# bobocode/lmono

Hardware: AMD Instinct MI355X
Metric: KITTI HDL-64 scans/sec (scanRegistration + laserOdometry) (higher is better)
Workload: dtype f32 features / f64 solve

## Files before the change

### lmono_amd/csrc/corr_flat.hip

```cpp
#include "batch.hpp"

namespace lmono {

#ifndef LMONO_CF_T
#define LMONO_CF_T 128
#endif
constexpr int kCfT = LMONO_CF_T;
constexpr int kCfBlocks = kMaxQueries / kCfT;
static_assert(kMaxQueries % kCfT == 0, "feature capacity must be a multiple of the workgroup size");
static_assert(kCfBlocks == kThinBlocks, "k_lm_solve skips the records of the workgroups a thinned lead-in pair does not run");
#ifndef LMONO_CF_PER
#define LMONO_CF_PER 6
#endif
#ifndef LMONO_CF_WAVES
#define LMONO_CF_WAVES 1
#endif
constexpr int kCfPer = LMONO_CF_PER;
constexpr int kCfPool = kCfT * kCfPer;
#ifndef LMONO_R0_PLANE
#define LMONO_R0_PLANE 0.25f
#define LMONO_R0_EDGE 0.7f
#endif
constexpr float kCfR0Edge = LMONO_R0_EDGE, kCfR0Plane = LMONO_R0_PLANE;
constexpr int kCfC = 4;
// ... 9 lines not shown
constexpr int kCfNnRounds = LMONO_CF_NN_ROUNDS, kCfWalkRounds = LMONO_CF_WALK_ROUNDS;
#ifndef LMONO_CF_MERGED
#define LMONO_CF_MERGED 0
#endif
#ifndef LMONO_WALK_TIGHT
#define LMONO_WALK_TIGHT 1
#endif

__device__ __forceinline__ unsigned int cf_request_line(int line, int b0, int nb, int owner) { return (unsigned int)line | ((unsigned int)b0 << 7) | ((unsigned int)nb << 16) | ((unsigned int)owner << 25); }
static_assert(kCfT <= 128 && kAzBins <= 511, "request packing");

struct CfRun {
    unsigned int start;
    unsigned int pre;
    unsigned short len;
    unsigned char owner;
    unsigned char tag;
};
static_assert(sizeof(CfRun) == 12, "run descriptor layout");

struct CfLds {
    float4 elev[2][66];
    int fge[2][66], lle[2][66];
    float4 q[kCfT];
    unsigned long long best[kCfT];
    unsigned long long same[kCfT], other[kCfT];
    int closest[kCfT], wlo[kCfT], whi[kCfT];
    unsigned int req[kCfPool];
    CfRun pool[kCfPool];
    int n_pool, n_cand, wsum[kCfT / 64];
    unsigned char wmode[kCfT];
};

__device__ __forceinline__ void cf_defer(unsigned int *wl, int c, int qi)
{
    const unsigned int slot = atomicAdd(wl, 1u);
    wl[1 + slot] = ((unsigned int)c << 12) | (unsigned int)qi;
}

struct CfArc { int a0, nb; };
__device__ __forceinline__ void cf_arc(float r, float rho, float th, CfArc &a)
{
    constexpr float kb = kAzBins / 6.28318531f;
    a.a0 = 0; a.nb = kAzBins;
    if (!(rho > r * 1.002f)) return;
    const float alpha = asin_upper(r / rho) + kArcSlackBins / kb;
    const int lo = (int)floorf((th - alpha) * kb), hi = (int)floorf((th + alpha) * kb);
    const int n = hi - lo + 1;
    if (n >= kAzBins) return;
    a.a0 = ((lo % kAzBins) + kAzBins) % kAzBins;
    a.nb = n;
}
__device__ __forceinline__ int cf_arc_pieces(const CfArc &a) { return a.a0 + a.nb > kAzBins ? 2 : 1; }
__device__ __forceinline__ void cf_post_line(unsigned int *req, int &slot, const CfArc &a, int line, int owner)
{
    const int n0 = min(a.nb, kAzBins - a.a0);
    req[slot++] = cf_request_line(line, a.a0, n0, owner);
    if (n0 < a.nb) req[slot++] = cf_request_line(line, 0, a.nb - n0, owner);
}

__device__ __forceinline__ int cf_first_line(const float4 *el, float ehi)
{
    int lo = 0, hi = 66;
    while (lo < hi) { const int mid = (lo + hi) >> 1; if (el[mid].z <= ehi) hi = mid; else lo = mid + 1; }
    return lo;
}
__device__ __forceinline__ int cf_last_line(const float4 *el, float elo)
{
    int lo = -1, hi = 65;
    while (lo < hi) { const int mid = (lo + hi + 1) >> 1; if (el[mid].w >= elo) lo = mid; else hi = mid - 1; }
// ... 136 lines not shown
                    const unsigned long long key = ((unsigned long long)__float_as_uint(d) << 32) | seq;
                    const bool is_other = sj > 0 ? (dv > 0) : (dv < 0);
                    m1 = (ok & is_other & (key < m1)) ? key : m1;
                    m0 = (ok & !is_other & (key < m0)) ? key : m0;
                }
            }
        }
        CF_STAMP(cf_acc[13])
        if (!more) break;
    }
    flush();
    CF_STAMP(cf_acc[14])
}

__global__ __launch_bounds__(kCfT, LMONO_CF_WAVES) void k_corr_flat(BatchView b, OdomView o, int step, int outer, unsigned int *wl, int defer_every, unsigned long long *stats)
{
    __shared__ CfLds L;
    const int xcd = blockIdx.x & 7, u = blockIdx.x >> 3;
    const int ci = o.chain0 + (u / kCfBlocks) * 8 + xcd;
    const int qb = u % kCfBlocks;
    if (ci >= o.chain1) return;
    const int c = o.clist ? o.clist[ci] : ci;
    int own;
    const int k = chain_scan(o, c, step, own);
    if (k < 0) return;
    if (lead_in_thinned(o, k, own) && qb % kThinStride != 0) return;
    const int tid = threadIdx.x;
    const int l = k - 1;
    const int n_sharp = b.feat_n[k * 4 + 0];
    const int nq = n_sharp + b.feat_n[k * 4 + 2];
    if (qb >= nq) return;
    const int qi = tid * kCfBlocks + qb;
    if (b.status[l] & (kStatusIrregularLines | kStatusDenseCell)) {
        if (qi < nq) cf_defer(wl, c, qi);
        return;
    }
    const bool edge = qi < n_sharp;
    const int cl = edge ? 0 : 1;
    const int n_edge_owner = n_sharp > qb ? (n_sharp - qb + kCfBlocks - 1) / kCfBlocks : 0;
    float4 fp = make_float4(0.f, 0.f, 0.f, 0.f);
    int *seed_c = o.seed ? o.seed + (size_t)c * kMaxQueries : nullptr;
    int sidx = -1;
    if (qi < nq) {
        fp = edge ? b.sharp[(size_t)k * kMaxSharp + qi] : b.flat[(size_t)k * kMaxFlat + (qi - n_sharp)];
        if (outer == 1 && seed_c) sidx = seed_c[qi];
    }
    int4 prev = make_int4(-1, -1, -1, 0);
    if (qi < nq && outer == 1 && seed_c && sidx >= 0) prev = ((const int4 *)o.corr + (size_t)c * kMaxQueries)[qi];
    for (int xx = tid; xx < 2 * 66; xx += kCfT) {
        const int tc = xx / 66, v = xx % 66;
        L.elev[tc][v] = b.lb_elev[(size_t)(l * 2 + tc) * 66 + v];
        L.fge[tc][v] = b.line_first_ge[(size_t)(l * 2 + tc) * 66 + v];
        L.lle[tc][v] = b.line_last_le[(size_t)(l * 2 + tc) * 66 + v];
    }
    const int n_last = b.feat_n[l * 4 + (edge ? 1 : 3)];
    const float4 *cloud = edge ? b.less_sharp + (size_t)l * kMaxLessSharp : b.less_flat + b.off[l];
    float4 sp = make_float4(0.f, 0.f, 0.f, 0.f);
    if (sidx >= 0 && sidx < n_last) sp = cloud[sidx]; else sidx = -1;
    const double *x = o.state + c * 8;
    double rx, ry, rz;
    quat_rotate(x, (double)fp.x, (double)fp.y, (double)fp.z, rx, ry, rz);
    const float qx = (float)(rx + x[4]), qy = (float)(ry + x[5]), qz = (float)(rz + x[6]);
    float sd = -1.0f;
    if (sidx >= 0) { const float d = dist2f(sp.x, sp.y, sp.z, qx, qy, qz); if (d < 24.0f) sd = d; }
    L.q[tid] = make_float4(qx, qy, qz, 0.f);
    L.best[tid] = ~0ull;
    const int *tg_c = b.lb_start + (size_t)(l * 2 + 0) * (kLineKeys + 1), *tg_s = b.lb_start + (size_t)(l * 2 + 1) * (kLineKeys + 1);
// ... 249 lines not shown
                const unsigned long long lim = pack_fu(r_now * r_now * 0.998f, 0u);
                if (other < lim && (edge || same < lim)) walking = false;
                else if (seeded) r_seed = -1.0f;
                else {
                    wpass++;
                    while (wpass < 4 && rad[wpass] <= rad[wpass - 1]) wpass++;
#if LMONO_WALK_TIGHT
                    if (other < thr && (edge || same < thr)) {
                        const float d = edge ? __uint_as_float((unsigned int)(other >> 32)) : fmaxf(__uint_as_float((unsigned int)(other >> 32)), __uint_as_float((unsigned int)(same >> 32)));
                        const float rt = sqrtf(d) * 1.002f + 1e-3f;
                        if (wpass < 4 && rt < rad[wpass] && d < 24.0f) r_seed = rt;
                    }
#endif
                }
            }
        }
        CF_STAMP(cf_acc[3])
        if (!__syncthreads_or(walking ? 1 : 0)) break;
    }
#endif
#ifdef LMONO_TILE_PROF
    {
        const int mr = __syncthreads_or(0) * 0 + my_rounds;
        __shared__ int s_maxr, s_sumr;
        if (tid == 0) { s_maxr = 0; s_sumr = 0; }
        __syncthreads();
        atomicMax(&s_maxr, mr); atomicAdd(&s_sumr, mr);
        __syncthreads();
        if (tid == 0) { cf_acc[17] = (unsigned long long)s_maxr; cf_acc[18] = (unsigned long long)s_sumr; }
    }
    if (tid == 0 && stats) { atomicAdd(&stats[1], 1ull); for (int i = 0; i < 20; i++) atomicAdd(&stats[2 + i], cf_acc[i]); }
#endif
    if (qi >= nq) return;
    if (deferred || walking) { cf_defer(wl, c, qi); return; }
    int4 rres = make_int4(-1, -1, -1, 0);
    int closest_out = -1;
    if (n_last > 0 && nn != ~0ull && (double)__uint_as_float((unsigned int)(nn >> 32)) < 25.0) {
        closest_out = closest;
        const int i_other = other < thr ? seq_to_index((unsigned int)(other & 0xffffffffull), closest) : -1;
        if (edge) { if (i_other >= 0) rres = make_int4(closest, i_other, -1, 1); }
        else {
            const int i_same = same < thr ? seq_to_index((unsigned int)(same & 0xffffffffull), closest) : -1;
            if (i_same >= 0 && i_other >= 0) rres = make_int4(closest, i_same, i_other, 2);
        }
    }
    ((int4 *)o.corr + (size_t)c * kMaxQueries)[qi] = rres;
    if (outer == 0 && seed_c) seed_c[qi] = closest_out;
    float4 A = make_float4(0.f, 0.f, 0.f, 0.f), B = A, C = A;
    if (rres.w != 0) { A = cloud[rres.x]; B = cloud[rres.y]; if (rres.z >= 0) C = cloud[rres.z]; }
    fp.w = __int_as_float(rres.w);
    float4 *rec = o.crec + ((size_t)c * kMaxQueries + qi) * 4;
    rec[0] = fp; rec[1] = A; rec[2] = B; rec[3] = C;
}

}
```

### lmono_amd/csrc/lidar_abi.hip

```cpp
#pragma once
constexpr int kListGrid = 256;

struct lmono_scan_batch {
    lmono_ctx *ctx = nullptr;
    int n_cap = 0;
    int64_t pts_cap = 0;
    int n_scans = 0;
    int64_t total = 0;
    int max_pts = 0;
    bool registered = false;
    bool grid_built = false;
    std::vector<int64_t> off_h;
    bool validation_pending = false;
    std::vector<void *> allocs;
    BatchView v{};
    int64_t *off_d = nullptr;
    float *in_owned = nullptr;
    hipEvent_t staged_ev = nullptr, in_free_ev = nullptr;
    int64_t staged_points = -1;
    std::vector<int> feat_h;
    int chains_cap = 0;
    double *state = nullptr, *incr = nullptr, *poses = nullptr, *xq = nullptr;
    int *corr = nullptr, *lm_info = nullptr, *corr_pair = nullptr, *seed = nullptr;
    float4 *crec = nullptr, *crec_pair = nullptr;
// ... 282 lines not shown
    switch (which) {
    case 0: HIP_TRY(c, hipMemcpy(&n, b->v.n_cloud + scan, sizeof(int), hipMemcpyDeviceToHost)); src = b->v.cloud + b->off_h[scan]; break;
    case 1: n = fn[0]; src = b->v.sharp + (size_t)scan * kMaxSharp; break;
    case 2: n = fn[1]; src = b->v.less_sharp + (size_t)scan * kMaxLessSharp; break;
    case 3: n = fn[2]; src = b->v.flat + (size_t)scan * kMaxFlat; break;
    default: n = fn[3]; src = b->v.less_flat + b->off_h[scan]; break;
    }
    if (n > cap) { c->err = "get_cloud: output capacity too small"; return LMONO_ECAPACITY; }
    if (n > 0) HIP_TRY(c, hipMemcpy(out_h, src, sizeof(float4) * n, hipMemcpyDeviceToHost));
    return n;
}

extern "C" int lmono_batch_get_curvature(lmono_ctx *c, lmono_scan_batch *b, int scan, float *curv_h, int32_t *label_h, int cap)
{
    if (!c || !b || !b->registered || scan < 0 || scan >= b->n_scans) return LMONO_EINVAL;
    HIP_TRY(c, hipStreamSynchronize(c->stream));
    int n = 0;
    HIP_TRY(c, hipMemcpy(&n, b->v.n_cloud + scan, sizeof(int), hipMemcpyDeviceToHost));
    if (n > cap) { c->err = "get_curvature: output capacity too small"; return LMONO_ECAPACITY; }
    if (curv_h && n > 0) HIP_TRY(c, hipMemcpy(curv_h, b->v.curv + b->off_h[scan], sizeof(float) * n, hipMemcpyDeviceToHost));
    if (label_h && n > 0) {
        std::vector<int8_t> tmp(n);
        HIP_TRY(c, hipMemcpy(tmp.data(), b->v.label + b->off_h[scan], n, hipMemcpyDeviceToHost));
        for (int i = 0; i < n; i++) label_h[i] = tmp[i];
    }
    return n;
}

static int ensure_odom_ws(lmono_ctx *c, lmono_scan_batch *b, int n_chains)
{
    if (n_chains <= b->chains_cap) return LMONO_OK;
    bool ok = dalloc(b, b->state, (size_t)n_chains * 8) && dalloc(b, b->corr, (size_t)n_chains * kMaxQueries * 4) &&
              dalloc(b, b->lm_info, (size_t)n_chains * 4) && dalloc(b, b->crec, (size_t)n_chains * kMaxQueries * 4) &&
              dalloc(b, b->seed, (size_t)n_chains * kMaxQueries) && dalloc(b, b->wl, 8 * ((size_t)n_chains * kMaxQueries + 1)) &&
              dalloc(b, b->ws, (size_t)n_chains * 8) && dalloc(b, b->resid_d, (size_t)n_chains) && dalloc(b, b->rstat, (size_t)n_chains * 4) &&
              dalloc(b, b->rcount, (size_t)n_chains + 2);
    if (!ok) { c->err = "odometry workspace: hipMalloc failed"; return LMONO_ENOMEM; }
    b->chains_cap = n_chains;
    return LMONO_OK;
}

static int ensure_grid(lmono_ctx *c, lmono_scan_batch *b)
{
    if (b->grid_built) return LMONO_OK;
#ifdef LMONO_DIAG_SEARCH
    hipLaunchKernelGGL(k_grid_build, dim3(b->n_scans, 1 + kGridPar), dim3(1024), kGridLds, c->stream, b->v);
    int rc = check_launch(c, "k_grid_build");
    if (rc) return rc;
    b->grid_built = true; b->v.has_grid = 1;
    return LMONO_OK;
#else
    c->err = "the hash-grid searches exist in the diagnostic build only (-DLMONO_DIAG_SEARCH)";
    return LMONO_EINVAL;
#endif
}

struct GroupFork {
    lmono_ctx *c; int G, g_own; bool forked = false;
    GroupFork(lmono_ctx *c_, int G_, int g_own_) : c(c_), G(G_), g_own(g_own_) {}
    int fork()
    {
        if (G <= 1) return LMONO_OK;
        for (int g = g_own; g < G; g++)
            if (!c->gstream[g]) {
                int lo = 0, hi = 0;
                if (c->odom_prio && hipDeviceGetStreamPriorityRange(&lo, &hi) == hipSuccess) HIP_TRY(c, hipStreamCreateWithPriority(&c->gstream[g], hipStreamNonBlocking, hi));
                else HIP_TRY(c, hipStreamCreateWithFlags(&c->gstream[g], hipStreamNonBlocking));
// ... 6 lines not shown
    }
    int join()
    {
        if (!forked) return LMONO_OK;
        forked = false;
        int rc = LMONO_OK;
        for (int g = g_own; g < G; g++) {
            if (hipEventRecord(c->gev[g + 1], c->gstream[g]) != hipSuccess || hipStreamWaitEvent(c->stream, c->gev[g + 1], 0) != hipSuccess) {
                (void)hipStreamSynchronize(c->gstream[g]);
                c->err = "odometry: joining a chain-group stream failed"; rc = LMONO_ENODEV;
            }
        }
        return rc;
    }
    ~GroupFork() { (void)join(); }
};

static int odom_groups(const lmono_ctx *c, int n_ch)
{
    constexpr int kMinChainsPerGroup = 32;
    int G = c->opt[LMONO_OPT_ODOM_STREAMS];
    G = G < 1 ? 1 : (G > 8 ? 8 : G);
    if (c->stream != nullptr && G > 3 && !c->many_queues) G = 3;
    while (G > 1 && n_ch / G < kMinChainsPerGroup) G--;
    if (c->opt[LMONO_OPT_CORR_TILE] != 3) G = 1;
    return G;
}

static int odom_launch_steps(lmono_ctx *c, lmono_scan_batch *b, const OdomView &o, int n_ch, int step_a, int step_b, int G, EvSet *es, int *ne)
{
    const int tile = c->opt[LMONO_OPT_CORR_TILE];
    hipStream_t st = c->stream;
    const int g_own = st == nullptr ? 1 : 0;
    const size_t wl_stride = (size_t)b->chains_cap * kMaxQueries + 1;
    auto kev = [&](int i) -> hipEvent_t {
        if (!es) return nullptr;
        while ((int)es->kev.size() <= i) { hipEvent_t e; if (hipEventCreate(&e) != hipSuccess) return nullptr; es->kev.push_back(e); }
        return es->kev[i];
    };
    GroupFork fork(c, G, g_own);
    int rc = fork.fork();
    if (rc) return rc;
    for (int step = step_a; step < step_b; step++) {
        for (int outer = 0; outer < 2; outer++) {
            for (int g = 0; g < G; g++) {
                hipStream_t sg = (G == 1 || g < g_own) ? st : c->gstream[g];
                OdomView og = o;
                og.chain0 = (int)((long long)g * n_ch / G); og.chain1 = (int)((long long)(g + 1) * n_ch / G);
                const int ng = og.chain1 - og.chain0;
                if (ng <= 0) continue;
                unsigned int *wlg = b->wl + g * wl_stride;
                hipEvent_t e0 = nullptr, e1 = nullptr, e2 = nullptr;
                if (g == 0 && es) { e0 = kev(*ne); e1 = kev(*ne + 1); e2 = kev(*ne + 2); }
                if (e0 && e1 && e2) (void)hipEventRecord(e0, sg);
                if (tile == 3) {
                    hipLaunchKernelGGL(k_corr_flat, dim3(8 * ((ng + 7) / 8) * kCfBlocks), dim3(kCfT), 0, sg, b->v, og, step, outer, wlg, c->opt[LMONO_OPT_DEFER_EVERY], c->stats_d);
                    hipLaunchKernelGGL(k_correspond_list, dim3(kListGrid), dim3(256), 0, sg, b->v, og, step, outer, (const unsigned int *)wlg, c->stats_d);
                }
#ifdef LMONO_DIAG_SEARCH
                else
                    hipLaunchKernelGGL(k_correspond, dim3(8 * ((ng + 7) / 8) * kCorrBlocks), dim3(256), 0, sg, b->v, og, step, outer);
#endif
                if (e0 && e1 && e2) (void)hipEventRecord(e1, sg);
                hipLaunchKernelGGL(k_lm_solve, dim3(ng), dim3(kLmT), kLmRecLds, sg, b->v, og, step, outer, tile ? wlg : (unsigned int *)nullptr);
                if (e0 && e1 && e2) { (void)hipEventRecord(e2, sg); *ne += 3; }
            }
        }
    }
    return fork.join();
}

static int odom_validate(lmono_ctx *c, lmono_scan_batch *b, OdomView o, bool ext, bool first_call, EvSet *es = nullptr, int *ne = nullptr)
{
    hipStream_t st = c->stream;
    const int n_chains = o.n_chains;
    lmono_boundary_report &R = b->brep;
    if (first_call) {
        R = lmono_boundary_report{};
        R.n_chains = n_chains; R.tol = o.tol;
        b->resid_h.assign(n_chains, 0.0); b->rerun_h.assign(n_chains, 0);
    }
    if (!b->rep_ev[0]) for (auto &e : b->rep_ev) HIP_TRY(c, hipEventCreate(&e));
    HIP_TRY(c, hipEventRecord(b->rep_ev[0], st));
    int max_len = 0;
    for (int ch = 0; ch < n_chains; ch++) { int s, e; chain_bounds(o.first, o.n_scans, n_chains, ch, s, e); max_len = e - s > max_len ? e - s : max_len; }
    const int tile = c->opt[LMONO_OPT_CORR_TILE];
    std::vector<int> rs((size_t)n_chains * 4);
    const int max_rounds = n_chains + 1;
    int still_flagged = 0;
    for (int round = 0; round <= max_rounds; round++) {
        const bool very_first = first_call && round == 0;
        hipLaunchKernelGGL(k_boundary_check, dim3(1), dim3(256), 0, st, o, very_first ? b->resid_d : (double *)nullptr, very_first ? 1 : 0, ext ? 1 : 0);
        unsigned int cnt[2] = { 0, 0 };
        HIP_TRY(c, hipMemcpyAsync(cnt, b->rcount, sizeof(cnt), hipMemcpyDeviceToHost, st));
        if (very_first) HIP_TRY(c, hipMemcpyAsync(b->resid_h.data(), b->resid_d, sizeof(double) * n_chains, hipMemcpyDeviceToHost, st));
        HIP_TRY(c, hipStreamSynchronize(st));
        if (very_first) {
            for (int ch = 0; ch < n_chains; ch++) R.max_resid = b->resid_h[ch] > R.max_resid ? b->resid_h[ch] : R.max_resid;
            if (R.max_resid >= 1e299) { c->err = "odometry: a chain boundary holds a NaN increment (a scan pair without a usable solution)"; return LMONO_ESCAN; }
        }
        const int nf = (int)cnt[0];
        still_flagged = nf;
        if (nf == 0 || round == max_rounds) break;
        R.flagged += nf; R.rounds += 1;
        OdomView orp = o;
        orp.repair = 1; orp.clist = (const int *)(b->rcount + 2); orp.lead_full = -1;
        const int G = odom_groups(c, nf);
        if (tile) for (int g = 0; g < G; g++) HIP_TRY(c, hipMemsetAsync(b->wl + g * ((size_t)b->chains_cap * kMaxQueries + 1), 0, sizeof(unsigned int), st));
        int done = 0, chunk = 3;
        while (done < max_len) {
            const int upto = done + chunk < max_len ? done + chunk : max_len;
            orp.step0 = 0;
            int rc = odom_launch_steps(c, b, orp, nf, done, upto, G, es, ne);
            if (rc) return rc;
            done = upto;
            HIP_TRY(c, hipMemcpyAsync(cnt, b->rcount, sizeof(cnt), hipMemcpyDeviceToHost, st));
            HIP_TRY(c, hipStreamSynchronize(st));
            if (cnt[1] == 0) break;
            chunk = chunk < 8 ? chunk * 2 : 8;
        }
    }
    HIP_TRY(c, hipEventRecord(b->rep_ev[1], st));
    HIP_TRY(c, hipMemcpyAsync(rs.data(), b->rstat, sizeof(int) * 4 * n_chains, hipMemcpyDeviceToHost, st));
    HIP_TRY(c, hipStreamSynchronize(st));
    float ms = 0.f;
    if (hipEventElapsedTime(&ms, b->rep_ev[0], b->rep_ev[1]) == hipSuccess) R.repair_ms += ms;
    R.pairs_rerun = 0; R.chains_rerun = 0;
    R.unresolved = still_flagged;
    for (int ch = 0; ch < n_chains; ch++) {
        b->rerun_h[ch] = rs[ch * 4 + 1];
        R.pairs_rerun += rs[ch * 4 + 1]; R.chains_rerun += rs[ch * 4 + 3] > 0 ? 1 : 0;
    }
    return check_launch(c, "boundary validation");
}

static OdomView odom_view(lmono_ctx *c, lmono_scan_batch *b, int n_chains, int lead, int first)
{
    OdomView o{};
    o.n_scans = b->n_scans; o.n_chains = n_chains; o.lead = lead; o.first = first; o.fixed_k = -1; o.chain0 = 0; o.chain1 = n_chains;
    o.lead_full = c->opt[LMONO_OPT_CORR_TILE] == 3 ? c->opt[LMONO_OPT_LEAD_FULL] : -1;
    o.state = b->state; o.corr = b->corr; o.incr = b->incr; o.lm_info = b->lm_info; o.crec = b->crec; o.seed = b->seed;
// ... 1 lines not shown
    o.tol = 1e-9 * (double)c->opt[LMONO_OPT_BOUNDARY_TOL];
    return o;
}

static int odom_run(lmono_ctx *c, lmono_scan_batch *b, int n_chains, int lead, int first, double *incr_d, double *poses_d, bool want_poses, bool validate = true)
{
    if (!c || !b || !b->registered || lead < 0 || first < 0 || first >= b->n_scans) return LMONO_EINVAL;
    const int n = b->n_scans;
    if (n_chains < 1) n_chains = 1;
    if (n_chains > n - first) n_chains = n - first;
    HIP_TRY(c, hipSetDevice(c->device));
    int rc = ensure_odom_ws(c, b, n_chains);
    if (rc) return rc;
    OdomView o = odom_view(c, b, n_chains, lead, first);
    b->last_chains = n_chains; b->last_lead = lead; b->last_first = first;
    int max_steps = 0;
    for (int ch = 0; ch < n_chains; ch++) {
        int s, e;
        chain_bounds(first, n, n_chains, ch, s, e);
        const int begin = s - lead > 0 ? s - lead : 0;
        const int steps = e - begin - 1;
        max_steps = steps > max_steps ? steps : max_steps;
    }
    hipStream_t st = c->stream;
    if (c->n_sets == 0 || c->sets[c->n_sets - 1].odom) c->ev = c->next_set();
    if (!c->ev) { c->err = "hipEventCreate failed"; return LMONO_ENODEV; }
    c->sets[c->n_sets - 1].odom = true;
    HIP_TRY(c, hipEventRecord(c->ev[8], st));
    const int ninit = n > n_chains ? n : n_chains;
    hipLaunchKernelGGL(k_odom_init, dim3((ninit + 255) / 256), dim3(256), 0, st, o);
    const int tile = c->opt[LMONO_OPT_CORR_TILE];
    if (tile != 3) { rc = ensure_grid(c, b); if (rc) return rc; }
    const int G = odom_groups(c, n_chains);
    if (tile) for (int g = 0; g < G; g++) HIP_TRY(c, hipMemsetAsync(b->wl + g * ((size_t)b->chains_cap * kMaxQueries + 1), 0, sizeof(unsigned int), st));
    EvSet &es = c->sets[c->n_sets - 1];
    int ne = 0;
    if (c->opt[LMONO_OPT_LEAD_SEED] > 0 && n_chains > 2 && lead >= 3 && max_steps > 1 && o.ws) {
        rc = odom_launch_steps(c, b, o, n_chains, 0, 1, G, &es, &ne);
        if (rc) return rc;
        hipLaunchKernelGGL(k_lead_seed_median, dim3((n_chains + 255) / 256), dim3(256), 0, st, o);
        hipLaunchKernelGGL(k_lead_seed_apply, dim3((n_chains + 255) / 256), dim3(256), 0, st, o);
        rc = odom_launch_steps(c, b, o, n_chains, 1, max_steps, G, &es, &ne);
    } else
        rc = odom_launch_steps(c, b, o, n_chains, 0, max_steps, G, &es, &ne);
    if (rc) return rc;
    es.n_kev = ne;
    b->brep = lmono_boundary_report{};
    b->brep.n_chains = n_chains;
    b->resid_h.assign((size_t)n_chains, 0.0); b->rerun_h.assign((size_t)n_chains, 0);
    b->validation_pending = !validate;
    if (validate && o.tol > 0.0 && n_chains > 1) { rc = odom_validate(c, b, o, false, true); if (rc) return rc; }
    if (want_poses) hipLaunchKernelGGL(k_pose_prefix, dim3(1), dim3(64), 0, st, (const double *)b->incr, b->poses, first, n);
    HIP_TRY(c, hipEventRecord(c->ev[9], st));
    rc = check_launch(c, "odometry kernels");
    if (rc) return rc;
    if (incr_d) HIP_TRY(c, hipMemcpyAsync(incr_d, b->incr, sizeof(double) * 7 * n, hipMemcpyDeviceToDevice, st));
    if (poses_d) HIP_TRY(c, hipMemcpyAsync(poses_d, b->poses, sizeof(double) * 7 * (n - first), hipMemcpyDeviceToDevice, st));
    return LMONO_OK;
}

extern "C" int lmono_odom_batch_d(lmono_ctx *c, lmono_scan_batch *b, int n_chains, int lead, double *incr_d, double *poses_d)
{
    return odom_run(c, b, n_chains, lead, 0, incr_d, poses_d, poses_d != nullptr);
}

extern "C" int lmono_odom_shard_d(lmono_ctx *c, lmono_scan_batch *b, int n_chains, int lead, int first_owned, double *incr_d)
{
// ... 110 lines not shown
    CP(v.line_first_ge, 2 * 66, (size_t)from * 2 * 66, (size_t)to * 2 * 66);
    CP(v.line_last_le, 2 * 66, (size_t)from * 2 * 66, (size_t)to * 2 * 66);
#undef CP
    return LMONO_OK;
}

extern "C" int lmono_odom_step(lmono_ctx *c, lmono_odom_stream *s, const float *xyzi, int n_points, int on_device, int use_warm_start,
                               double *q_last_curr, double *t_last_curr, double *q_w_curr, double *t_w_curr, int32_t *info)
{
    if (!c || !s || s->ctx != c || !xyzi || n_points < 0) return LMONO_EINVAL;
    if (n_points > s->cap_pts) { c->err = "lmono_odom_step: more points than the stream's slots hold"; return LMONO_ECAPACITY; }
    if (use_warm_start && (!q_last_curr || !t_last_curr)) return LMONO_EINVAL;
    HIP_TRY(c, hipSetDevice(c->device));
    lmono_scan_batch *b = s->batch;
    hipStream_t st = c->stream;
    int next = s->frame == 0 ? 1 : s->slot + 1;
    if (next >= s->n_slots) {
        int rc = stream_copy_last(c, b, s->slot, 0);
        if (rc) return rc;
        next = 1;
    }
    float *dst = s->in_d + (size_t)next * s->cap_pts * 4;
    if (n_points > 0) HIP_TRY(c, hipMemcpyAsync(dst, xyzi, (size_t)n_points * 16, on_device ? hipMemcpyDeviceToDevice : hipMemcpyHostToDevice, st));
    if (n_points < s->cap_pts) HIP_TRY(c, hipMemsetAsync(dst + (size_t)n_points * 4, 0xff, (size_t)(s->cap_pts - n_points) * 16, st));
    int rc = scanreg_launch(c, b, next, 1, n_points, n_points > 0 ? n_points : 1);
    if (rc) return rc;
    b->feat_h.clear();
    int iters[4] = { 0, 0, 0, 0 };
    if (s->frame > 0) {
        if (use_warm_start) { for (int i = 0; i < 4; i++) s->para[i] = q_last_curr[i]; for (int i = 0; i < 3; i++) s->para[4 + i] = t_last_curr[i]; }
        HIP_TRY(c, hipMemcpyAsync(b->state, s->para, sizeof(double) * 8, hipMemcpyHostToDevice, st));
        OdomView o = odom_view(c, b, 1, 0, 0);
        o.fixed_k = next; o.ws = nullptr; o.lead_full = -1;
        HIP_TRY(c, hipMemsetAsync(b->wl, 0, sizeof(unsigned int), st));
        rc = odom_launch_steps(c, b, o, 1, 0, 1, 1, nullptr, nullptr);
        if (rc) return rc;
        HIP_TRY(c, hipMemcpyAsync(s->para, b->state, sizeof(double) * 8, hipMemcpyDeviceToHost, st));
        HIP_TRY(c, hipMemcpyAsync(iters, b->lm_info, sizeof(iters), hipMemcpyDeviceToHost, st));
    }
    int fn[6] = { 0, 0, 0, 0, 0, 0 };
    HIP_TRY(c, hipMemcpyAsync(fn, b->v.n_cloud + next, sizeof(int), hipMemcpyDeviceToHost, st));
    HIP_TRY(c, hipMemcpyAsync(fn + 1, b->v.feat_n + next * 4, sizeof(int) * 4, hipMemcpyDeviceToHost, st));
    HIP_TRY(c, hipMemcpyAsync(fn + 5, b->v.status + next, sizeof(int), hipMemcpyDeviceToHost, st));
    HIP_TRY(c, hipStreamSynchronize(st));
    if (s->frame > 0) {
        const double *q = s->para, *t = s->para + 4;
        const double ux = s->q_w[0], uy = s->q_w[1], uz = s->q_w[2], w = s->q_w[3];
        const double uvx = 2.0 * (uy * t[2] - uz * t[1]), uvy = 2.0 * (uz * t[0] - ux * t[2]), uvz = 2.0 * (ux * t[1] - uy * t[0]);
        s->t_w[0] += t[0] + w * uvx + (uy * uvz - uz * uvy);
        s->t_w[1] += t[1] + w * uvy + (uz * uvx - ux * uvz);
        s->t_w[2] += t[2] + w * uvz + (ux * uvy - uy * uvx);
        const double bx = q[0], by = q[1], bz = q[2], bw = q[3];
        const double nw = w * bw - ux * bx - uy * by - uz * bz, nx = w * bx + ux * bw + uy * bz - uz * by;
        const double ny = w * by + uy * bw + uz * bx - ux * bz, nz = w * bz + uz * bw + ux * by - uy * bx;
        s->q_w[0] = nx; s->q_w[1] = ny; s->q_w[2] = nz; s->q_w[3] = nw;
    }
    if (q_last_curr) for (int i = 0; i < 4; i++) q_last_curr[i] = s->para[i];
    if (t_last_curr) for (int i = 0; i < 3; i++) t_last_curr[i] = s->para[4 + i];
    if (q_w_curr) for (int i = 0; i < 4; i++) q_w_curr[i] = s->q_w[i];
    if (t_w_curr) for (int i = 0; i < 3; i++) t_w_curr[i] = s->t_w[i];
    if (info) { for (int i = 0; i < 6; i++) info[i] = fn[i]; info[6] = (iters[0] << 8) | iters[1]; info[7] = iters[3]; }
    s->slot = next; s->frame++;
    if (fn[5] & kStatusRingOverflow) { c->err = "lmono_odom_step: a ring holds more than LMONO_RING_CAP points"; return LMONO_ESCAN; }
    return LMONO_OK;
}

extern "C" int lmono_odom_stream_scan(lmono_odom_stream *s, lmono_scan_batch **batch, int *scan)
{
    if (!s || s->frame == 0) return LMONO_EINVAL;
    if (batch) *batch = s->batch;
    if (scan) *scan = s->slot;
    return LMONO_OK;
}

extern "C" int lmono_odom_correspond(lmono_ctx *c, lmono_scan_batch *b, int scan, const double q[4], const double t[3],
                                     int32_t *corr_h, int cap)
{
    if (!c || !b || !b->registered || scan < 1 || scan >= b->n_scans || !q || !t || !corr_h) return LMONO_EINVAL;
    HIP_TRY(c, hipSetDevice(c->device));
    double x[8] = { q[0], q[1], q[2], q[3], t[0], t[1], t[2], 0.0 };
    HIP_TRY(c, hipStreamSynchronize(c->stream));
    HIP_TRY(c, hipMemcpy(b->xq, x, sizeof(x), hipMemcpyHostToDevice));
    int fn[4];
    HIP_TRY(c, hipMemcpy(fn, b->v.feat_n + scan * 4, sizeof(fn), hipMemcpyDeviceToHost));
    const int nq = fn[0] + fn[2];
    if (nq > cap) { c->err = "odom_correspond: output capacity too small"; return LMONO_ECAPACITY; }
    OdomView o{};
    o.n_scans = b->n_scans; o.n_chains = 1; o.lead = 0; o.fixed_k = scan; o.chain0 = 0; o.chain1 = 1; o.lead_full = -1;
    o.state = b->xq; o.corr = b->corr_pair; o.incr = nullptr; o.lm_info = nullptr; o.crec = b->crec_pair; o.seed = nullptr;
    int rc;
    if (c->opt[LMONO_OPT_CORR_TILE] != 3) { rc = ensure_grid(c, b); if (rc) return rc; }
    if (c->opt[LMONO_OPT_CORR_TILE]) {
        rc = ensure_odom_ws(c, b, 1);
        if (rc) return rc;
        HIP_TRY(c, hipMemsetAsync(b->wl, 0, sizeof(unsigned int), c->stream));
        hipLaunchKernelGGL(k_corr_flat, dim3(8 * kCfBlocks), dim3(kCfT), 0, c->stream, b->v, o, 0, 0, b->wl, c->opt[LMONO_OPT_DEFER_EVERY], c->stats_d);
        hipLaunchKernelGGL(k_correspond_list, dim3(kListGrid), dim3(256), 0, c->stream, b->v, o, 0, 0, (const unsigned int *)b->wl, c->stats_d);
    }
#ifdef LMONO_DIAG_SEARCH
    else
        hipLaunchKernelGGL(k_correspond, dim3(8 * kCorrBlocks), dim3(256), 0, c->stream, b->v, o, 0, 0);
#endif
    rc = check_launch(c, "k_correspond");
    if (rc) return rc;
    HIP_TRY(c, hipStreamSynchronize(c->stream));
    if (nq > 0) HIP_TRY(c, hipMemcpy(corr_h, b->corr_pair, sizeof(int) * 4 * nq, hipMemcpyDeviceToHost));
    return nq;
}

extern "C" int lmono_pose_prefix_d(lmono_ctx *c, const double *incr_d, int first, int n, double *poses_d)
{
    if (!c || !incr_d || !poses_d || first < 0 || n <= first) return LMONO_EINVAL;
    HIP_TRY(c, hipSetDevice(c->device));
    hipLaunchKernelGGL(k_pose_prefix, dim3(1), dim3(64), 0, c->stream, incr_d, poses_d, first, n);
    return check_launch(c, "k_pose_prefix");
}

extern "C" int lmono_pose_rebase_d(lmono_ctx *c, const double *bases_d, int n_bases, double *poses_d, int n)
{
    if (!c || !poses_d || n <= 0 || n_bases < 0 || (n_bases > 0 && !bases_d)) return LMONO_EINVAL;
    HIP_TRY(c, hipSetDevice(c->device));
    hipLaunchKernelGGL(k_pose_rebase, dim3((n + 255) / 256), dim3(256), 0, c->stream, bases_d, n_bases, poses_d, n);
    return check_launch(c, "k_pose_rebase");
}
```

### lmono_amd/csrc/odometry.hip

```cpp
#include "batch.hpp"

namespace lmono {

constexpr float kCell = 1.0f;
constexpr float kInvCell = 1.0f;
constexpr int kMaxShell = 6;
constexpr int kCoordOff = 1 << 20;
constexpr int kRunMaxCount = 32767;
__device__ __forceinline__ int pack_run(int start, int count) { return start | (count << 17); }

__device__ __forceinline__ unsigned long long cell_key(int cx, int cy, int cz)
{
    return ((unsigned long long)(unsigned int)(cx + kCoordOff) << 42) |
           ((unsigned long long)(unsigned int)(cy + kCoordOff) << 21) |
           (unsigned long long)(unsigned int)(cz + kCoordOff);
}
__device__ __forceinline__ unsigned int hash_key(unsigned long long k)
{
    const unsigned int cz = (unsigned int)(k & 0x1fffffull), cy = (unsigned int)((k >> 21) & 0x1fffffull), cx = (unsigned int)(k >> 42);
    unsigned int h = (cx * 73856093u) ^ (cy * 19349663u) ^ (cz * 83492791u);
    h ^= h >> 15;
    return h;
}

// ... 865 lines not shown
constexpr int kCorrBlocks = kMaxQueries / 8;

#ifdef LMONO_DIAG_SEARCH
__global__ __launch_bounds__(256, 8) void k_correspond(BatchView b, OdomView o, int step, int outer)
{
    const int xcd = blockIdx.x & 7, u = blockIdx.x >> 3;
    const int c = o.chain0 + (u / kCorrBlocks) * 8 + xcd;
    const int qblock = u % kCorrBlocks;
    if (c >= o.chain1) return;
    const int lane = threadIdx.x & 63;
    const int gl = threadIdx.x & (kGroup - 1), gbase = lane & ~(kGroup - 1);
    int own;
    const int k = chain_scan(o, c, step, own);
    if (k < 0) return;
    const int n_sharp = b.feat_n[k * 4 + 0];
    const int nq = n_sharp + b.feat_n[k * 4 + 2];
    const double *x = o.state + c * 8;
    int4 *corr = (int4 *)o.corr + (size_t)c * kMaxQueries;
    const int l = k - 1;
    if (b.status[l] & (kStatusIrregularLines | kStatusDenseCell)) {
        for (int t = 0; t < 2; t++) {
            const int qi = qblock * 8 + (threadIdx.x >> 6) * 2 + t;
            if (qi >= nq) break;
            correspond_wave(b, o, c, k, qi, lane);
        }
        return;
    }
    const int qi = qblock * 8 + (threadIdx.x >> 5);
    if (qi >= nq) return;
    correspond_group(b, o, c, k, qi, outer, gl, gbase);
}
#endif

__global__ __launch_bounds__(256, 4) void k_correspond_list(BatchView b, OdomView o, int step, int outer, const unsigned int *wl, unsigned long long *stats)
{
    const unsigned int n = wl[0];
    if (blockIdx.x == 0 && threadIdx.x == 0 && stats && n) atomicAdd(&stats[0], (unsigned long long)n);
    const int lane = threadIdx.x & 63;
    const int gl = threadIdx.x & (kGroup - 1), gbase = lane & ~(kGroup - 1);
    for (unsigned int it = blockIdx.x * 8 + (threadIdx.x >> 5); it < n; it += gridDim.x * 8) {
        const unsigned int e = wl[1 + it];
        const int c = (int)(e >> 12), qi = (int)(e & 4095u);
        int own;
        const int k = chain_scan(o, c, step, own);
        if (k < 0 || (b.status[k - 1] & (kStatusIrregularLines | kStatusDenseCell))) continue;
        correspond_group(b, o, c, k, qi, outer, gl, gbase);
    }
    for (unsigned int it = blockIdx.x * 4 + (threadIdx.x >> 6); it < n; it += gridDim.x * 4) {
        const unsigned int e = wl[1 + it];
        const int c = (int)(e >> 12), qi = (int)(e & 4095u);
        int own;
        const int k = chain_scan(o, c, step, own);
        if (k < 0 || !(b.status[k - 1] & (kStatusIrregularLines | kStatusDenseCell))) continue;
        correspond_wave(b, o, c, k, qi, lane);
    }
}

constexpr int kLmT = 256;
constexpr int kLmW = kLmT / 64;
struct LmAcc { double H[21]; double g[6]; double cost; };

__device__ __forceinline__ void quat_rotate_fma(const double *q, double vx, double vy, double vz, double &ox, double &oy, double &oz)
{
#pragma clang fp contract(fast)
    const double ux = q[0], uy = q[1], uz = q[2], w = q[3];
    const double uvx = 2.0 * (uy * vz - uz * vy);
    const double uvy = 2.0 * (uz * vx - ux * vz);
    const double uvz = 2.0 * (ux * vy - uy * vx);
    ox = vx + w * uvx + (uy * uvz - uz * uvy);
    oy = vy + w * uvy + (uz * uvx - ux * uvz);
    oz = vz + w * uvz + (ux * uvy - uy * uvx);
}

__device__ __forceinline__ void accumulate_row(LmAcc &a, const double *J, double r)
{
#pragma clang fp contract(fast)
    int t = 0;
#pragma unroll
    for (int i = 0; i < 6; i++) {
        a.g[i] += J[i] * r;
#pragma unroll
        for (int j = i; j < 6; j++) a.H[t++] += J[i] * J[j];
    }
}

__device__ __forceinline__ void huber(double s, double &rho0, double &rho1)
{
    const double a = 0.1, bb = 0.1 * 0.1;
// ... 258 lines not shown
            else ev.template run<true>(cand);
            const double cand_cost = s_sum[27];
            double sn = 0.0;
            for (int i = 0; i < 7; i++) sn += (x[i] - cand[i]) * (x[i] - cand[i]);
            sn = sqrt(sn);
            if (sn <= parameter_tol * (x_norm + parameter_tol)) break;
            if (fabs(x_cost - cand_cost) <= function_tol * x_cost) break;
            const double rel = (x_cost - cand_cost) / model_change;
            if (rel > min_rel_decrease) {
                for (int i = 0; i < 7; i++) x[i] = cand[i];
                if (last) break;
                x_norm = norm7(x);
                x_cost = cand_cost;
                __syncthreads();
                if (tid < 28) s_cur[tid] = s_sum[tid];
                __syncthreads();
                const double tt = 2.0 * rel - 1.0;
                double den = 1.0 - tt * tt * tt;
                if (den < 1.0 / 3.0) den = 1.0 / 3.0;
                radius = radius / den;
                if (radius > max_radius) radius = max_radius;
                decrease_factor = 2.0; reuse_diagonal = false;
                gmax = 0.0;
                for (int i = 0; i < 6; i++) gmax = fmax(gmax, fabs(s_cur[21 + i]));
                if (gmax <= gradient_tol) break;
            } else {
                radius = radius / decrease_factor; decrease_factor *= 2.0; reuse_diagonal = true;
            }
            if (radius <= min_radius) break;
        }
    }
}

__global__ __launch_bounds__(kLmT) void k_lm_solve(BatchView b, OdomView o, int step, int outer, unsigned int *wl_reset)
{
    const int c = o.clist ? o.clist[o.chain0 + blockIdx.x] : o.chain0 + (int)blockIdx.x;
    if (wl_reset && blockIdx.x == 0 && threadIdx.x == 0) wl_reset[0] = 0u;
    int s;
    const int k = chain_scan(o, c, step, s);
    if (k < 0) return;
    __shared__ double s_red[kLmW][28], s_sum[28], s_cur[28];
    __shared__ int s_used[kLmW];
    const int tid = threadIdx.x, lane = tid & 63, wave = tid >> 6;
    const int n_edge = b.feat_n[k * 4 + 0], nq = n_edge + b.feat_n[k * 4 + 2];
    const float4 *crec = o.crec + (size_t)c * kMaxQueries * 4;
    extern __shared__ __align__(16) float4 s_rec[];
    int n_used = 0;
    {
        double2 *sp = (double2 *)s_rec;
        const bool thin = lead_in_thinned(o, k, s);
        for (int qi = tid; qi < nq; qi += kLmT) {
            float4 cp = crec[qi * 4];
            const float4 A = crec[qi * 4 + 1], B = crec[qi * 4 + 2], Cc = crec[qi * 4 + 3];
            if (thin && (qi % kThinBlocks) % kThinStride != 0) cp.w = 0.f;
            double P[6] = { 0.0, 0.0, 0.0, 0.0, 0.0, 0.0 };
            if (__float_as_int(cp.w) != 0) { stage_block(cp, A, B, Cc, P); n_used++; }
            s_rec[qi] = cp;
            sp[kMaxQueries + qi] = make_double2(P[0], P[1]);
            sp[2 * kMaxQueries + qi] = make_double2(P[2], P[3]);
            sp[3 * kMaxQueries + qi] = make_double2(P[4], P[5]);
        }
    }
    __syncthreads();
    double x[7];
    for (int i = 0; i < 7; i++) x[i] = o.state[c * 8 + i];

    LmRecEval ev{ s_rec, n_edge, nq, s_red, s_sum };
    int iter = 0;
    ev.run<true>(x);
    n_used = wave_sum_i(n_used);
    if (lane == 0) s_used[wave] = n_used;
    __syncthreads();
    n_used = 0;
// ... 180 lines not shown
```

Measured before the change: 120,000.

## Fold deferred work-list serving into the LM solve kernel via double-buffered heads

Removes the separate k_correspond_list launch from the per-step odometry loop. Each k_lm_solve workgroup now serves the deferred correspondence entries belonging to its own chain before solving. The work-list counter is double-buffered by outer parity so the solve kernel can reset the other head without a race. This saves one kernel launch per iteration. In exchange, every LM workgroup scans the whole work list and filters by chain, which costs more when many queries are deferred.

```diff
diff --git a/lmono_amd/csrc/corr_flat.hip b/lmono_amd/csrc/corr_flat.hip
--- a/lmono_amd/csrc/corr_flat.hip
+++ b/lmono_amd/csrc/corr_flat.hip
@@ -65,10 +65,10 @@
     unsigned char wmode[kCfT];
 };
 
-__device__ __forceinline__ void cf_defer(unsigned int *wl, int c, int qi)
+__device__ __forceinline__ void cf_defer(unsigned int *wl, int outer, int c, int qi)
 {
-    const unsigned int slot = atomicAdd(wl, 1u);
-    wl[1 + slot] = ((unsigned int)c << 12) | (unsigned int)qi;
+    const unsigned int slot = atomicAdd(wl + (outer & 1), 1u);
+    wl[kWlHeads + slot] = ((unsigned int)c << 12) | (unsigned int)qi;
 }
 
 struct CfArc { int a0, nb; };
@@ -271,7 +271,7 @@
     if (qb >= nq) return;
     const int qi = tid * kCfBlocks + qb;
     if (b.status[l] & (kStatusIrregularLines | kStatusDenseCell)) {
-        if (qi < nq) cf_defer(wl, c, qi);
+        if (qi < nq) cf_defer(wl, outer, c, qi);
         return;
     }
     const bool edge = qi < n_sharp;
@@ -587,7 +587,7 @@
     if (tid == 0 && stats) { atomicAdd(&stats[1], 1ull); for (int i = 0; i < 20; i++) atomicAdd(&stats[2 + i], cf_acc[i]); }
 #endif
     if (qi >= nq) return;
-    if (deferred || walking) { cf_defer(wl, c, qi); return; }
+    if (deferred || walking) { cf_defer(wl, outer, c, qi); return; }
     int4 rres = make_int4(-1, -1, -1, 0);
     int closest_out = -1;
     if (n_last > 0 && nn != ~0ull && (double)__uint_as_float((unsigned int)(nn >> 32)) < 25.0) {
diff --git a/lmono_amd/csrc/lidar_abi.hip b/lmono_amd/csrc/lidar_abi.hip
--- a/lmono_amd/csrc/lidar_abi.hip
+++ b/lmono_amd/csrc/lidar_abi.hip
@@ -338,7 +338,7 @@
     if (n_chains <= b->chains_cap) return LMONO_OK;
     bool ok = dalloc(b, b->state, (size_t)n_chains * 8) && dalloc(b, b->corr, (size_t)n_chains * kMaxQueries * 4) &&
               dalloc(b, b->lm_info, (size_t)n_chains * 4) && dalloc(b, b->crec, (size_t)n_chains * kMaxQueries * 4) &&
-              dalloc(b, b->seed, (size_t)n_chains * kMaxQueries) && dalloc(b, b->wl, 8 * ((size_t)n_chains * kMaxQueries + 1)) &&
+              dalloc(b, b->seed, (size_t)n_chains * kMaxQueries) && dalloc(b, b->wl, 8 * ((size_t)n_chains * kMaxQueries + kWlHeads)) &&
               dalloc(b, b->ws, (size_t)n_chains * 8) && dalloc(b, b->resid_d, (size_t)n_chains) && dalloc(b, b->rstat, (size_t)n_chains * 4) &&
               dalloc(b, b->rcount, (size_t)n_chains + 2);
     if (!ok) { c->err = "odometry workspace: hipMalloc failed"; return LMONO_ENOMEM; }
@@ -411,7 +411,7 @@
     const int tile = c->opt[LMONO_OPT_CORR_TILE];
     hipStream_t st = c->stream;
     const int g_own = st == nullptr ? 1 : 0;
-    const size_t wl_stride = (size_t)b->chains_cap * kMaxQueries + 1;
+    const size_t wl_stride = (size_t)b->chains_cap * kMaxQueries + kWlHeads;
     auto kev = [&](int i) -> hipEvent_t {
         if (!es) return nullptr;
         while ((int)es->kev.size() <= i) { hipEvent_t e; if (hipEventCreate(&e) != hipSuccess) return nullptr; es->kev.push_back(e); }
@@ -432,16 +432,14 @@
                 hipEvent_t e0 = nullptr, e1 = nullptr, e2 = nullptr;
                 if (g == 0 && es) { e0 = kev(*ne); e1 = kev(*ne + 1); e2 = kev(*ne + 2); }
                 if (e0 && e1 && e2) (void)hipEventRecord(e0, sg);
-                if (tile == 3) {
+                if (tile == 3)
                     hipLaunchKernelGGL(k_corr_flat, dim3(8 * ((ng + 7) / 8) * kCfBlocks), dim3(kCfT), 0, sg, b->v, og, step, outer, wlg, c->opt[LMONO_OPT_DEFER_EVERY], c->stats_d);
-                    hipLaunchKernelGGL(k_correspond_list, dim3(kListGrid), dim3(256), 0, sg, b->v, og, step, outer, (const unsigned int *)wlg, c->stats_d);
-                }
 #ifdef LMONO_DIAG_SEARCH
                 else
                     hipLaunchKernelGGL(k_correspond, dim3(8 * ((ng + 7) / 8) * kCorrBlocks), dim3(256), 0, sg, b->v, og, step, outer);
 #endif
                 if (e0 && e1 && e2) (void)hipEventRecord(e1, sg);
-                hipLaunchKernelGGL(k_lm_solve, dim3(ng), dim3(kLmT), kLmRecLds, sg, b->v, og, step, outer, tile ? wlg : (unsigned int *)nullptr);
+                hipLaunchKernelGGL(k_lm_solve, dim3(ng), dim3(kLmT), kLmRecLds, sg, b->v, og, step, outer, tile == 3 ? wlg : (unsigned int *)nullptr, c->stats_d);
                 if (e0 && e1 && e2) { (void)hipEventRecord(e2, sg); *ne += 3; }
             }
         }
@@ -485,7 +483,7 @@
         OdomView orp = o;
         orp.repair = 1; orp.clist = (const int *)(b->rcount + 2); orp.lead_full = -1;
         const int G = odom_groups(c, nf);
-        if (tile) for (int g = 0; g < G; g++) HIP_TRY(c, hipMemsetAsync(b->wl + g * ((size_t)b->chains_cap * kMaxQueries + 1), 0, sizeof(unsigned int), st));
+        if (tile) for (int g = 0; g < G; g++) HIP_TRY(c, hipMemsetAsync(b->wl + g * ((size_t)b->chains_cap * kMaxQueries + kWlHeads), 0, kWlHeads * sizeof(unsigned int), st));
         int done = 0, chunk = 3;
         while (done < max_len) {
             const int upto = done + chunk < max_len ? done + chunk : max_len;
@@ -553,7 +551,7 @@
     const int tile = c->opt[LMONO_OPT_CORR_TILE];
     if (tile != 3) { rc = ensure_grid(c, b); if (rc) return rc; }
     const int G = odom_groups(c, n_chains);
-    if (tile) for (int g = 0; g < G; g++) HIP_TRY(c, hipMemsetAsync(b->wl + g * ((size_t)b->chains_cap * kMaxQueries + 1), 0, sizeof(unsigned int), st));
+    if (tile) for (int g = 0; g < G; g++) HIP_TRY(c, hipMemsetAsync(b->wl + g * ((size_t)b->chains_cap * kMaxQueries + kWlHeads), 0, kWlHeads * sizeof(unsigned int), st));
     EvSet &es = c->sets[c->n_sets - 1];
     int ne = 0;
     if (c->opt[LMONO_OPT_LEAD_SEED] > 0 && n_chains > 2 && lead >= 3 && max_steps > 1 && o.ws) {
@@ -730,7 +728,7 @@
         HIP_TRY(c, hipMemcpyAsync(b->state, s->para, sizeof(double) * 8, hipMemcpyHostToDevice, st));
         OdomView o = odom_view(c, b, 1, 0, 0);
         o.fixed_k = next; o.ws = nullptr; o.lead_full = -1;
-        HIP_TRY(c, hipMemsetAsync(b->wl, 0, sizeof(unsigned int), st));
+        HIP_TRY(c, hipMemsetAsync(b->wl, 0, kWlHeads * sizeof(unsigned int), st));
         rc = odom_launch_steps(c, b, o, 1, 0, 1, 1, nullptr, nullptr);
         if (rc) return rc;
         HIP_TRY(c, hipMemcpyAsync(s->para, b->state, sizeof(double) * 8, hipMemcpyDeviceToHost, st));
@@ -791,7 +789,7 @@
     if (c->opt[LMONO_OPT_CORR_TILE]) {
         rc = ensure_odom_ws(c, b, 1);
         if (rc) return rc;
-        HIP_TRY(c, hipMemsetAsync(b->wl, 0, sizeof(unsigned int), c->stream));
+        HIP_TRY(c, hipMemsetAsync(b->wl, 0, kWlHeads * sizeof(unsigned int), c->stream));
         hipLaunchKernelGGL(k_corr_flat, dim3(8 * kCfBlocks), dim3(kCfT), 0, c->stream, b->v, o, 0, 0, b->wl, c->opt[LMONO_OPT_DEFER_EVERY], c->stats_d);
         hipLaunchKernelGGL(k_correspond_list, dim3(kListGrid), dim3(256), 0, c->stream, b->v, o, 0, 0, (const unsigned int *)b->wl, c->stats_d);
     }
diff --git a/lmono_amd/csrc/odometry.hip b/lmono_amd/csrc/odometry.hip
--- a/lmono_amd/csrc/odometry.hip
+++ b/lmono_amd/csrc/odometry.hip
@@ -921,28 +921,39 @@
 }
 #endif
 
-__global__ __launch_bounds__(256, 4) void k_correspond_list(BatchView b, OdomView o, int step, int outer, const unsigned int *wl, unsigned long long *stats)
-{
-    const unsigned int n = wl[0];
-    if (blockIdx.x == 0 && threadIdx.x == 0 && stats && n) atomicAdd(&stats[0], (unsigned long long)n);
+constexpr int kWlHeads = 2;
+__device__ __forceinline__ void serve_work_list(const BatchView &b, const OdomView &o, int step, int outer, const unsigned int *wl, unsigned int n,
+                                                int only_chain, unsigned int first, unsigned int stride)
+{
+    const unsigned int *ent = wl + kWlHeads;
     const int lane = threadIdx.x & 63;
     const int gl = threadIdx.x & (kGroup - 1), gbase = lane & ~(kGroup - 1);
-    for (unsigned int it = blockIdx.x * 8 + (threadIdx.x >> 5); it < n; it += gridDim.x * 8) {
-        const unsigned int e = wl[1 + it];
+    const unsigned int ng = blockDim.x >> 5, nw = blockDim.x >> 6;
+    for (unsigned int it = first * ng + (threadIdx.x >> 5); it < n; it += stride * ng) {
+        const unsigned int e = ent[it];
         const int c = (int)(e >> 12), qi = (int)(e & 4095u);
+        if (only_chain >= 0 && c != only_chain) continue;
         int own;
         const int k = chain_scan(o, c, step, own);
         if (k < 0 || (b.status[k - 1] & (kStatusIrregularLines | kStatusDenseCell))) continue;
         correspond_group(b, o, c, k, qi, outer, gl, gbase);
     }
-    for (unsigned int it = blockIdx.x * 4 + (threadIdx.x >> 6); it < n; it += gridDim.x * 4) {
-        const unsigned int e = wl[1 + it];
+    for (unsigned int it = first * nw + (threadIdx.x >> 6); it < n; it += stride * nw) {
+        const unsigned int e = ent[it];
         const int c = (int)(e >> 12), qi = (int)(e & 4095u);
+        if (only_chain >= 0 && c != only_chain) continue;
         int own;
         const int k = chain_scan(o, c, step, own);
         if (k < 0 || !(b.status[k - 1] & (kStatusIrregularLines | kStatusDenseCell))) continue;
         correspond_wave(b, o, c, k, qi, lane);
     }
+}
+
+__global__ __launch_bounds__(256, 4) void k_correspond_list(BatchView b, OdomView o, int step, int outer, const unsigned int *wl, unsigned long long *stats)
+{
+    const unsigned int n = wl[outer & 1];
+    if (blockIdx.x == 0 && threadIdx.x == 0 && stats && n) atomicAdd(&stats[0], (unsigned long long)n);
+    serve_work_list(b, o, step, outer, wl, n, -1, blockIdx.x, gridDim.x);
 }
 
 constexpr int kLmT = 256;
@@ -1267,13 +1278,24 @@
     }
 }
 
-__global__ __launch_bounds__(kLmT) void k_lm_solve(BatchView b, OdomView o, int step, int outer, unsigned int *wl_reset)
+__global__ __launch_bounds__(kLmT) void k_lm_solve(BatchView b, OdomView o, int step, int outer, unsigned int *wl, unsigned long long *stats)
 {
     const int c = o.clist ? o.clist[o.chain0 + blockIdx.x] : o.chain0 + (int)blockIdx.x;
-    if (wl_reset && blockIdx.x == 0 && threadIdx.x == 0) wl_reset[0] = 0u;
+    unsigned int n_list = 0;
+    if (wl) {
+        n_list = __builtin_amdgcn_readfirstlane(wl[outer & 1]);
+        if (blockIdx.x == 0 && threadIdx.x == 0) {
+            wl[(outer + 1) & 1] = 0u;
+            if (stats && n_list) atomicAdd(&stats[0], (unsigned long long)n_list);
+        }
+    }
     int s;
     const int k = chain_scan(o, c, step, s);
     if (k < 0) return;
+    if (n_list) {
+        serve_work_list(b, o, step, outer, wl, n_list, c, 0u, 1u);
+        __syncthreads();
+    }
     __shared__ double s_red[kLmW][28], s_sum[28], s_cur[28];
     __shared__ int s_used[kLmW];
     const int tid = threadIdx.x, lane = tid & 63, wave = tid >> 6;
```

New measurement: 120,000 (median of 2 runs). Within noise of the previous version (+0.0%).
